# lorenzrichter/path-space-PDE-solver

Measured on AMD Instinct MI355X. Metric: trajectory-timesteps/sec (K*N/s), d=100 HJB log-variance training iteration, higher is better.
Workload: dtype f32 (f16x3 split products: every matrix product as three f16 MFMAs, fp32 accumulate; state / sums fp32)

## Files before the change

path-space-pde-solver_amd/csrc/hjb_basis_kernels.h:

```cpp
#pragma once
#include <hip/hip_runtime.h>

namespace psp {

constexpr int kBasisThreads = 256, kBasisRows = 4;
inline int basis_lds_bytes(int d) { return (kBasisRows * (d + 1) + d * d) * 4; }

template <bool TRANSPOSE>
__global__ __launch_bounds__(kBasisThreads) void hjb_basis_w1_kernel(const float* src, float* dst, const float* __restrict__ B,
                                                                     int d, int H, long long n) {
    extern __shared__ __attribute__((aligned(16))) float lds[];
    const int tid = threadIdx.x, nthr = blockDim.x;
    const int h0 = blockIdx.x * kBasisRows;
    const int rows = (H - h0) < kBasisRows ? (H - h0) : kBasisRows;
    const int nw = rows * (d + 1);
    const float* wsrc = src + (long long)h0 * (d + 1);
    float* wdst = dst + (long long)h0 * (d + 1);
    float* w = lds;
    float* m = lds + kBasisRows * (d + 1);
    for (int idx = tid; idx < nw; idx += nthr) w[idx] = wsrc[idx];
    for (int idx = tid; idx < d * d; idx += nthr) {
        const int i = idx / d, j = idx - i * d;
        m[TRANSPOSE ? j * d + i : idx] = B[idx];
    }
    if (dst != src) {
        const long long base = (long long)H * (d + 1);
        for (long long idx = base + (long long)blockIdx.x * nthr + tid; idx < n; idx += (long long)gridDim.x * nthr) dst[idx] = src[idx];
    }
    __syncthreads();
    for (int idx = tid; idx < nw; idx += nthr) {
        const int h = idx / (d + 1), c = idx - h * (d + 1);
        float v = w[idx];
        if (c > 0) {
            const float* row = w + h * (d + 1) + 1;
            const int j = c - 1;
            v = 0.f;
            for (int i = 0; i < d; ++i) v = fmaf(row[i], m[i * d + j], v);
        }
        wdst[idx] = v;
    }
}

template <bool TRANSPOSE>
inline hipError_t launch_basis_w1(const float* src, float* dst, const float* B, int d, int H, long long n, hipStream_t s) {
    const int grid = (H + kBasisRows - 1) / kBasisRows;
    hipLaunchKernelGGL((hjb_basis_w1_kernel<TRANSPOSE>), dim3(grid), dim3(kBasisThreads), basis_lds_bytes(d), s, src, dst, B, d, H, n);
    return hipGetLastError();
}

}
```

path-space-pde-solver_amd/csrc/hjb_kernels.h:

```cpp
#pragma once
#include <cstdlib>
#include <type_traits>
#include <hip/hip_runtime.h>
#include <stdint.h>

namespace psp {

typedef float f32x4 __attribute__((ext_vector_type(4)));

struct HjbArgs {
    const float* params;
    const float* x0;
    const float* y0;
    const float* xi;
    float* path;
    float* D;
    float* XN;
    double* fwd_partial;
    const float* drift;
    const float* sigma;
    const float* runcost;
    const float* term;
    const double* sums;
    float* grad_partial;
// ... 493 lines not shown
        split4c(last, b4h, b4l);
#pragma unroll
        for (int mb = 0; mb < MB; ++mb) {
            const f16x4* p = reinterpret_cast<const f16x4*>(wlds + mb * SG::per_mb + NS * 512) + lane;
            const f16x4 a_hi = p[0], a_lo = p[64];
            acc[mb] = __builtin_amdgcn_mfma_f32_16x16x16f16(a_hi, b4h, acc[mb], 0, 0, 0);
            corr[mb] = __builtin_amdgcn_mfma_f32_16x16x16f16(a_hi, b4l, corr[mb], 0, 0, 0);
            corr[mb] = __builtin_amdgcn_mfma_f32_16x16x16f16(a_lo, b4h, corr[mb], 0, 0, 0);
        }
    }
#pragma unroll
    for (int mb = 0; mb < MB; ++mb) acc[mb] = acc[mb] + kSplitInv * corr[mb];
}

__device__ __forceinline__ float qsum(float v) {
    v += __shfl_xor(v, 16);
    v += __shfl_xor(v, 32);
    return v;
}
__device__ __forceinline__ float jsumf(float v) {
    v += __shfl_xor(v, 1);
    v += __shfl_xor(v, 2);
    v += __shfl_xor(v, 4);
    v += __shfl_xor(v, 8);
    return v;
}
__device__ __forceinline__ double jsum(double v) {
    v += __shfl_xor(v, 1);
    v += __shfl_xor(v, 2);
    v += __shfl_xor(v, 4);
    v += __shfl_xor(v, 8);
    return v;
}

__device__ __forceinline__ float tanh_f32(float x) {
    const float e = __builtin_amdgcn_exp2f(fabsf(x) * 2.8853900817779268f);
    const float big = fmaf(-2.0f, __builtin_amdgcn_rcpf(e + 1.0f), 1.0f);
    return copysignf(big, x);
}
__device__ __forceinline__ f32x4 tanh4(f32x4 v) {
    f32x4 o;
    o[0] = tanh_f32(v[0]); o[1] = tanh_f32(v[1]); o[2] = tanh_f32(v[2]); o[3] = tanh_f32(v[3]);
    return o;
}

__device__ __forceinline__ f32x4 relu4n(f32x4 v) {
    f32x4 o;
    o[0] = v[0] < 0.f ? 0.f : v[0]; o[1] = v[1] < 0.f ? 0.f : v[1]; o[2] = v[2] < 0.f ? 0.f : v[2]; o[3] = v[3] < 0.f ? 0.f : v[3];
    return o;
}

template <int D, int H>
struct Geo {
    static constexpr int DB = cdiv(D, 16), HB = cdiv(H, 16);
    static constexpr int KSD = cdiv(D, 4), KSH = cdiv(H, 4);
    static constexpr int oW1 = 0, ob1 = H * (D + 1), oW2 = ob1 + H, ob2 = oW2 + H * H, oW3 = ob2 + H,
                         ob3 = oW3 + D * H, P = ob3 + D;
    static constexpr int fW1 = 0, fW2 = fW1 + HB * KSD * 64, fW3 = fW2 + HB * KSH * 64,
                         fVec = fW3 + DB * KSH * 64;
    static constexpr int vb1 = fVec, vw1t = vb1 + HB * 16, vb2 = vw1t + HB * 16, vb3 = vb2 + HB * 16,
                         vdr = vb3 + DB * 16, vrun = vdr + DB * 16, vterm = vrun + DB * 16,
                         fRed = vterm + DB * 16;
    static constexpr int fA = fRed + 64;
    static constexpr int fB_dense_off = DB * KSD * 64;
    static constexpr int xW1 = 0, xW2 = xW1 + SplitGeo<KSD, DB>::floats(HB), xW3 = xW2 + SplitGeo<KSH, HB>::floats(HB),
                         xVec = xW3 + SplitGeo<KSH, HB>::floats(DB), xA = xVec + (fA - fVec);
    static constexpr int xB_dense_off = SplitGeo<KSD, DB>::floats(DB);
    static int fwd_x3_lds_floats(int drift_kind, int sigma_kind) {
        return xA + (drift_kind == DRIFT_DENSE ? xB_dense_off : 0) + (sigma_kind == SIGMA_DENSE ? xB_dense_off : 0);
    }
    static int fwd_lds_floats(int drift_kind, int sigma_kind) {
        return fA + (drift_kind == DRIFT_DENSE ? fB_dense_off : 0) + (sigma_kind == SIGMA_DENSE ? fB_dense_off : 0);
    }
    static constexpr int pX = 0, pH1 = 4 * DB * 64, pH2 = pH1 + 4 * HB * 64, pXi = pH2 + 4 * HB * 64, PB = pXi + 4 * DB * 64;
    static constexpr int WH = (HB >= 4) ? 4 : (HB >= 2 ? 2 : 1);
    static constexpr int WD = 4 / WH;
    static constexpr int NIB = cdiv(HB, WH);
    static constexpr int NOBD = cdiv(DB, WD);
    static constexpr int NOBH = cdiv(HB, WD);
    static constexpr int EXB = KSD * 64 + 4 * HB * 64;
    static int bwd2_lds_floats() { return HB * KSD * 64 + 2 * 4 * EXB; }
};

template <int D, int H, int MODE = 0, int FAST_ = 0>
__global__ __launch_bounds__(512) void hjb_fwd_kernel(const HjbArgs a) {
    PSP_COND_EXIT(a);
    constexpr bool FAST = FAST_ != 0, SPEC = FAST_ >= 2;
    const int k_drift = SPEC ? (int)DRIFT_DENSE : a.drift_kind;
    const int k_sigma = FAST_ == 3 ? (int)SIGMA_IDENT : SPEC ? (int)SIGMA_DENSE : a.sigma_kind;
    const int k_run = SPEC ? (int)RUN_ZERO : a.runcost_kind, k_loss = SPEC ? (int)LOSS_LOGVAR : a.loss_kind;
    const int k_store = a.store_path;
    const bool k_adaptive = SPEC ? true : (a.adaptive != 0);
    const uint32_t iter_now = a.iter_dev ? *a.iter_dev : a.iter;
    using G = Geo<D, H>;
    constexpr int DB = G::DB, HB = G::HB, KSD = G::KSD, KSH = G::KSH;
    constexpr bool BF16 = MODE == 1, X3 = MODE == 2;
    constexpr int oW1 = X3 ? G::xW1 : G::fW1, oW2 = X3 ? G::xW2 : G::fW2, oW3 = X3 ? G::xW3 : G::fW3;
    constexpr int VEC = X3 ? G::xVec : G::fVec;
    constexpr int VSH = VEC - G::fVec;
    extern __shared__ __attribute__((aligned(16))) float lds[];
    const int tid = threadIdx.x, nthr = blockDim.x;
    const int lane = tid & 63, wave = tid >> 6, nwave = nthr >> 6;
    const int j = lane & 15, q = lane >> 4;

    const float* __restrict__ P = a.params;
    auto stage_net = [&](float* dst, int MB, int KS, int INB, auto src) {
        if constexpr (BF16) stage_aop_bf16(dst, MB, (INB + 1) / 2, tid, nthr, src);
        else stage_aop(dst, MB, KS, tid, nthr, src);
    };
    auto w1src = [&](int row, int col) { return (row < H && col < D) ? P[G::oW1 + row * (D + 1) + 1 + col] : 0.f; };
    auto w2src = [&](int row, int col) { return (row < H && col < H) ? P[G::oW2 + row * H + col] : 0.f; };
    auto w3src = [&](int row, int col) { return (row < D && col < H) ? P[G::oW3 + row * H + col] : 0.f; };
    if constexpr (X3) {
        stage_aop_x3<KSD, DB>(lds + oW1, HB, tid, nthr, w1src);
        stage_aop_x3<KSH, HB>(lds + oW2, HB, tid, nthr, w2src);
        stage_aop_x3<KSH, HB>(lds + oW3, DB, tid, nthr, w3src);
    } else {
        stage_net(lds + oW1, HB, KSD, DB, w1src);
        stage_net(lds + oW2, HB, KSH, HB, w2src);
        stage_net(lds + oW3, DB, KSH, HB, w3src);
    }
    float* ldsA = lds + G::fA + VSH;
    float* ldsB = ldsA + (k_drift == DRIFT_DENSE ? (X3 ? G::xB_dense_off : G::fB_dense_off) : 0);
    if (k_drift == DRIFT_DENSE) {
        const float dt = a.dt;
        const float* __restrict__ A = a.drift;
        auto asrc = [&](int row, int col) { return (row < D && col < D) ? dt * A[row * D + col] : 0.f; };
        if constexpr (X3) stage_aop_x3<KSD, DB>(ldsA, DB, tid, nthr, asrc);
        else stage_aop(ldsA, DB, KSD, tid, nthr, asrc);
    }
    if (k_sigma == SIGMA_DENSE) {
        const float* __restrict__ B = a.sigma;
        auto bsrc = [&](int row, int col) { return (row < D && col < D) ? B[row * D + col] : 0.f; };
        if constexpr (X3) stage_aop_x3<KSD, DB>(ldsB, DB, tid, nthr, bsrc);
        else stage_aop(ldsB, DB, KSD, tid, nthr, bsrc);
    }
    stage_vec(lds + VSH + G::vb1, HB, tid, nthr, [&](int f) { return f < H ? P[G::ob1 + f] : 0.f; });
    stage_vec(lds + VSH + G::vw1t, HB, tid, nthr, [&](int f) { return f < H ? P[G::oW1 + f * (D + 1)] : 0.f; });
    stage_vec(lds + VSH + G::vb2, HB, tid, nthr, [&](int f) { return f < H ? P[G::ob2 + f] : 0.f; });
    stage_vec(lds + VSH + G::vb3, DB, tid, nthr, [&](int f) { return f < D ? P[G::ob3 + f] : 0.f; });
    stage_vec(lds + VSH + G::vdr, DB, tid, nthr, [&](int f) {
        return (f < D && (k_drift == DRIFT_DIAG || k_drift == DRIFT_DWELL)) ? a.drift[f] : 0.f; });
    stage_vec(lds + VSH + G::vrun, DB, tid, nthr, [&](int f) {
        return (f < D && k_run == RUN_DIAGQ) ? a.runcost[f] : 0.f; });
    stage_vec(lds + VSH + G::vterm, DB, tid, nthr, [&](int f) { return f < D ? a.term[f] : 0.f; });
    __syncthreads();

    const int t16 = blockIdx.x * nwave + wave;
    const bool wave_valid = t16 < a.ntile16;
    const int k = t16 * 16 + j;
    const bool kvalid = wave_valid && k < a.K_local;
    const uint32_t kglob = (uint32_t)(a.k_offset + k);
    const float dt = a.dt, sqdt = a.sqdt;

    const float store_cxi = SPEC ? 1.f : ((k_store == 3) ? 0.f : 1.f);
    const float store_cz = SPEC ? 0.f : ((k_store == 3) ? 1.f : (k_store == 2 ? -a.sqdt : (k_adaptive ? 0.f : a.sqdt)));
    const bool do_store = FAST ? true : (k_store != 0);
    double sD = 0.0, sD2 = 0.0;
    if (wave_valid) {
        const f32x4* vecs0 = reinterpret_cast<const f32x4*>(lds + VEC) + q;
        const f32x4* vterm = vecs0 + (G::vterm - G::fVec) / 4;

        f32x4 X[DB];
#pragma unroll
        for (int b = 0; b < DB; ++b) {
#pragma unroll
            for (int r = 0; r < 4; ++r) {
                const int f = 16 * b + 4 * r + q;
                const float v = a.x0[(size_t)(kvalid ? k : 0) * a.x0_stride + (f < D ? f : D - 1)];
                X[b][r] = (f < D && kvalid) ? v : 0.f;
            }
        }
        float Y = a.y0 ? a.y0[0] : 0.f;
        float Fsum = 0.f, ULsum = 0.f;
#ifdef PSP_STAMPS
        unsigned long long stamps[8] = {0, 0, 0, 0, 0, 0, 0, 0};
#endif

        for (int n = 0; n < a.N; ++n) {
            PSP_STAMP(fs0);
            float tn = (float)n * dt;
            if constexpr (!FAST) { if (a.tfeat) tn = a.tfeat[n]; }
            const f32x4* vecs = opaque(vecs0);
            const f32x4* vb1 = vecs + (G::vb1 - G::fVec) / 4;
            const f32x4* vw1t = vecs + (G::vw1t - G::fVec) / 4;
            const f32x4* vb2 = vecs + (G::vb2 - G::fVec) / 4;
            const f32x4* vb3 = vecs + (G::vb3 - G::fVec) / 4;
            const f32x4* vdr = vecs + (G::vdr - G::fVec) / 4;
            const f32x4* vrun = vecs + (G::vrun - G::fVec) / 4;
            float* pblk = a.path + ((size_t)n * a.ntile16 + t16) * (size_t)G::PB + lane;
            auto x_store = [&](int u, int NU) __attribute__((always_inline)) {
                if (do_store) {
#pragma unroll
                    for (int ks = 0; ks < 4 * DB; ++ks)
                        if (ks >= u * (4 * DB) / NU && ks < (u + 1) * (4 * DB) / NU)
                            PSP_PATH_STORE(pblk + (G::pX / 64 + ks) * 64, X[ks >> 2][ks & 3]);
                }
            };
            if (!X3 && do_store) {
#pragma unroll
                for (int ks = 0; ks < 4 * DB; ++ks) PSP_PATH_STORE(pblk + (G::pX / 64 + ks) * 64, X[ks >> 2][ks & 3]);
            }
            f32x4 h1[HB];
#pragma unroll
            for (int m = 0; m < HB; ++m) h1[m] = vb1[m * 4] + tn * vw1t[m * 4];
            f32x4 Tn[DB];
            const bool early_drift = X3 && k_drift == DRIFT_DENSE;
            if constexpr (X3) {
                if (k_drift == DRIFT_DENSE) {
                    f16x8 xh[DB / 2 > 0 ? DB / 2 : 1], xl[DB / 2 > 0 ? DB / 2 : 1];
                    constexpr int NU1 = (DB / 2) * HB, NU2 = (DB / 2) * DB;
                    split_panel8<DB>(X, xh, xl);
                    gemm_Txs<HB, KSD, DB, 2>(h1, lds + oW1, xh, xl, X[DB - 1], lane, [&](int u) __attribute__((always_inline)) { x_store(u, NU1 + NU2); });
#pragma unroll
                    for (int b = 0; b < DB; ++b) Tn[b] = X[b];
                    gemm_Txs<DB, KSD, DB, 2>(Tn, ldsA, xh, xl, X[DB - 1], lane, [&](int u) __attribute__((always_inline)) { x_store(NU1 + u, NU1 + NU2); });
                    if constexpr (NU1 + NU2 == 0) x_store(0, 1);
                } else {
                    constexpr int NU1 = (DB / 2) * HB;
                    gemm_Tx<HB, KSD, DB, 2>(h1, lds + oW1, X, lane, [&](int u) __attribute__((always_inline)) { x_store(u, NU1); });
                    if constexpr (NU1 == 0) x_store(0, 1);
                }
            }
            else if constexpr (BF16) gemm_Tb<HB, DB>(h1, lds + oW1, X, lane);
            else gemm_T<HB, KSD, DB>(h1, lds + oW1, X, lane);
            PSP_STAMP(fs1);
#pragma unroll
            for (int m = 0; m < HB; ++m) h1[m] = tanh4(h1[m]);
            PSP_STAMP(fs2);
            f32x4 h2[HB];
#pragma unroll
            for (int m = 0; m < HB; ++m) h2[m] = vb2[m * 4];
            constexpr int NUH2 = (HB / 2) * HB, NUH3 = (HB / 2) * DB;
            constexpr bool PREGEN = X3 && FAST && (NUH2 + NUH3 > 0);
            [[maybe_unused]] f32x4 xig[PREGEN ? DB : 1];
            [[maybe_unused]] uint32_t pc0 = 0, pc1 = 0, pc2 = 0, pc3 = 0;
            constexpr int NSPC = kPhiloxRounds + 1;
            auto philox_slice = [&](int sidx) __attribute__((always_inline)) {
                const int b = sidx / NSPC, sub = sidx % NSPC;
                if (sub == 0) { pc0 = kglob; pc1 = (uint32_t)n; pc2 = (uint32_t)(4 * b + q); pc3 = iter_now; }
                if (sub < kPhiloxRounds) {
                    philox_round(pc0, pc1, pc2, pc3, a.seed_lo + (uint32_t)sub * 0x9E3779B9u, a.seed_hi + (uint32_t)sub * 0xBB67AE85u);
                    asm volatile("" : "+v"(pc0), "+v"(pc1), "+v"(pc2), "+v"(pc3));
                } else {
                    const uint32_t rr[4] = {pc0, pc1, pc2, pc3};
                    f32x4 xi = normal4(rr);
                    if (16 * b + 16 > D) {
#pragma unroll
                        for (int r = 0; r < 4; ++r) if (16 * b + 4 * r + q >= D) xi[r] = 0.f;
                    }
                    asm volatile("" : "+v"(xi));
                    xig[b < DB ? b : 0] = xi;
                }
            };
            auto philox_portion = [&](int u) __attribute__((always_inline)) {
                if constexpr (PREGEN) {
#pragma unroll
                    for (int sidx = 0; sidx < NSPC * DB; ++sidx)
                        if (sidx >= u * (NSPC * DB) / (NUH2 + NUH3) && sidx < (u + 1) * (NSPC * DB) / (NUH2 + NUH3)) philox_slice(sidx);
                }
            };
            auto h_store = [&](const f32x4 (&h)[HB], int slot, int u, int NU) __attribute__((always_inline)) {
                if (do_store) {
#pragma unroll
                    for (int ks = 0; ks < 4 * HB; ++ks)
                        if (ks >= u * (4 * HB) / NU && ks < (u + 1) * (4 * HB) / NU)
                            PSP_PATH_STORE(pblk + (slot / 64 + ks) * 64, h[ks >> 2][ks & 3]);
                }
            };
            if constexpr (X3) {
                gemm_Tx<HB, KSH, HB, 2>(h2, lds + oW2, h1, lane, [&](int u) __attribute__((always_inline)) { h_store(h1, G::pH1, u, NUH2); philox_portion(u); });
                if constexpr (NUH2 == 0) h_store(h1, G::pH1, 0, 1);
            }
            else if constexpr (BF16) gemm_Tb<HB, HB>(h2, lds + oW2, h1, lane);
            else gemm_T<HB, KSH, HB>(h2, lds + oW2, h1, lane);
#pragma unroll
            for (int m = 0; m < HB; ++m) h2[m] = tanh4(h2[m]);
            if (!X3 && do_store) {
#pragma unroll
                for (int ks = 0; ks < 4 * HB; ++ks) {
                    PSP_PATH_STORE(pblk + (G::pH1 / 64 + ks) * 64, h1[ks >> 2][ks & 3]);
                    PSP_PATH_STORE(pblk + (G::pH2 / 64 + ks) * 64, h2[ks >> 2][ks & 3]);
                }
            }
            f32x4 Z[DB];
#pragma unroll
            for (int m = 0; m < DB; ++m) Z[m] = vb3[m * 4];
            if constexpr (X3) {
                gemm_Tx<DB, KSH, HB, 2>(Z, lds + oW3, h2, lane, [&](int u) __attribute__((always_inline)) { h_store(h2, G::pH2, u, NUH3); philox_portion(NUH2 + u); });
                if constexpr (NUH3 == 0) h_store(h2, G::pH2, 0, 1);
            }
            else if constexpr (BF16) gemm_Tb<DB, HB>(Z, lds + oW3, h2, lane);
            else gemm_T<DB, KSH, HB>(Z, lds + oW3, h2, lane);
            PSP_STAMP(fs3);

            float S = 0.f, Pz = 0.f, UL = 0.f;
#pragma unroll
            for (int b = 0; b < DB; ++b) {
                f32x4 xi;
                if constexpr (PREGEN) {
                    xi = xig[b];
                } else if (FAST || a.noise_mode == NOISE_PHILOX) {
                    xi = philox_block(kglob, (uint32_t)n, (uint32_t)(4 * b + q), iter_now, a.seed_lo, a.seed_hi);
                } else {
                    const float* xrow = a.xi + ((size_t)(n + 1) * a.K_local + (kvalid ? k : 0)) * D;
#pragma unroll
                    for (int r = 0; r < 4; ++r) {
                        const int f = 16 * b + 4 * r + q;
                        const float v = xrow[f < D ? f : D - 1];
                        xi[r] = (f < D && kvalid) ? v : 0.f;
                    }
                }
                if (16 * b + 16 > D) {
#pragma unroll
                    for (int r = 0; r < 4; ++r) if (16 * b + 4 * r + q >= D) xi[r] = 0.f;
                }
                if (do_store && k_store != 4) {
                    const f32x4 wv = store_cxi * xi + store_cz * Z[b];
#pragma unroll
                    for (int r = 0; r < 4; ++r) PSP_PATH_STORE(pblk + (G::pXi / 64 + 4 * b + r) * 64, wv[r]);
                }
#pragma unroll
                for (int r = 0; r < 4; ++r) {
                    S = fmaf(Z[b][r], Z[b][r], S);
                    Pz = fmaf(Z[b][r], xi[r], Pz);
                }
                if (!FAST && a.uref) {
                    const float* ur = a.uref + (size_t)n * D;
#pragma unroll
                    for (int r = 0; r < 4; ++r) {
                        const int f = 16 * b + 4 * r + q;
                        const float e = (f < D) ? Z[b][r] + ur[f < D ? f : D - 1] : 0.f;
                        UL = fmaf(e, e, UL);
                    }
                }
                Z[b] = k_adaptive ? (sqdt * xi - dt * Z[b]) : (sqdt * xi);
            }
            ULsum = fmaf(UL, dt, ULsum);
            S = qsum(S);
            Pz = qsum(Pz);
            PSP_STAMP(fs4);

            if (!early_drift) {
#pragma unroll
                for (int b = 0; b < DB; ++b) Tn[b] = X[b];
            }
            if (k_drift == DRIFT_DENSE) {
                if constexpr (!X3) gemm_T<DB, KSD, DB>(Tn, ldsA, X, lane);
            } else if (k_drift == DRIFT_DIAG) {
#pragma unroll
                for (int b = 0; b < DB; ++b) Tn[b] += dt * (vdr[b * 4] * X[b]);
            } else if (k_drift == DRIFT_DWELL) {
#pragma unroll
                for (int b = 0; b < DB; ++b) Tn[b] -= dt * (4.0f * vdr[b * 4] * (X[b] * (X[b] * X[b] - 1.0f)));
            }
            if (k_sigma == SIGMA_DENSE) {
                if constexpr (X3) gemm_Tx<DB, KSD, DB>(Tn, ldsB, Z, lane);
                else gemm_T<DB, KSD, DB>(Tn, ldsB, Z, lane);
            } else if (k_sigma == SIGMA_SCALE) {
#pragma unroll
                for (int b = 0; b < DB; ++b) Tn[b] += a.sigma_scale * Z[b];
            } else {
#pragma unroll
                for (int b = 0; b < DB; ++b) Tn[b] += Z[b];
            }
#pragma unroll
            for (int b = 0; b < DB; ++b) X[b] = Tn[b];
            PSP_STAMP(fs5);

            float fX = 0.f;
            if (k_run == RUN_DIAGQ) {
#pragma unroll
                for (int b = 0; b < DB; ++b) {
                    const f32x4 pv = vrun[b * 4];
#pragma unroll
                    for (int r = 0; r < 4; ++r) fX = fmaf(pv[r] * X[b][r], X[b][r], fX);
                }
                fX = qsum(fX);
            }
            if (k_loss == LOSS_RELENT) {
                Y = Y - (0.5f * S + fX) * dt;
            } else {
                const float drift_y = k_adaptive ? (fX - 0.5f * S) : (fX + 0.5f * S);
                Y = Y + drift_y * dt + Pz * sqdt;
            }
            Fsum = fmaf(fX, dt, Fsum);
            PSP_STAMP(fs6);
            PSP_ACC(0, fs1, fs0);
            PSP_ACC(1, fs2, fs1);
            PSP_ACC(2, fs3, fs2);
            PSP_ACC(3, fs4, fs3);
            PSP_ACC(4, fs5, fs4);
            PSP_ACC(5, fs6, fs5);
            PSP_ACC(6, fs6, fs0);
        }
#ifdef PSP_STAMPS
        if (a.dbg && lane == 0) {
            stamps[7] = (unsigned long long)a.N;
            for (int i = 0; i < 8; ++i) a.dbg[((size_t)blockIdx.x * 8 + wave) * 8 + i] = stamps[i];
// ... 493 lines not shown
```

path-space-pde-solver_amd/csrc/hjbx_kernels.h:

```cpp
#pragma once
#include "hjb_kernels.h"

namespace psp {

template <int D, int H>
struct GeoX {
    using G = Geo<D, H>;
    static constexpr int DB = G::DB, HB = G::HB, KSD = G::KSD, KSH = G::KSH;
    static constexpr int T3 = 0, T2 = T3 + SplitGeo<KSD, DB>::floats(HB), EX = T2 + SplitGeo<KSH, HB>::floats(HB);
    static constexpr int hG = 0, hGl = hG + D * 32, hZ2 = hGl + D * 32, hZ2l = hZ2 + HB * 512, hZ1 = hZ2l + HB * 512,
                         hZ1l = hZ1 + HB * 512, PAIRH = hZ1l + HB * 512;
    static constexpr int RS = 16 * DB + 3 * 16 * HB;
    static constexpr int NX = cdiv(DB, 4);
    static constexpr int NT = DB + 2 * HB;
    static_assert(4 * RS <= 4 * (PAIRH / 2), "bias sums reuse the exchange area");
    static constexpr int GS = EX + 4 * (PAIRH / 2);
    static int lds_floats() { return GS + 12; }
};

template <int NB>
__device__ __forceinline__ void split_panel(const f32x4 (&v)[NB], f16x4 (&hi)[NB], f16x4 (&lo)[NB]) {
#pragma unroll
    for (int b = 0; b < NB; ++b) {
        if ((NB & 1) && b == NB - 1) split4c(v[b], hi[b], lo[b]);
        else split4(v[b], hi[b], lo[b]);
    }
}

template <int MB, int KS, int INB>
__device__ __forceinline__ void gemm_Txp(f32x4 (&acc)[MB], const float* wlds, const f16x4 (&hi)[INB], const f16x4 (&lo)[INB],
                                         float last, int lane) {
    using SG = SplitGeo<KS, INB>;
    constexpr int NS = SG::NS;
    lane = opaque_i(lane);
    f32x4 corr[MB];
#pragma unroll
    for (int mb = 0; mb < MB; ++mb) corr[mb] = f32x4{0.f, 0.f, 0.f, 0.f};
    if constexpr (NS > 0) {
        const f16x8* tbl = reinterpret_cast<const f16x8*>(wlds) + lane;
        constexpr int NU = NS * MB, CU = 1, NCH = cdiv(NU, CU);
        f16x8 ah[2][CU], al[2][CU];
#pragma unroll
        for (int kk = 0; kk < CU; ++kk)
            if (kk < NU) {
                ah[0][kk] = tbl[((kk % MB) * SG::per_mb + (kk / MB) * 512) / 4];
                al[0][kk] = tbl[((kk % MB) * SG::per_mb + (kk / MB) * 512) / 4 + 64];
            }
#pragma unroll
        for (int c = 0; c < NCH; ++c) {
            if (c + 1 < NCH) {
#pragma unroll
                for (int kk = 0; kk < CU; ++kk) {
                    const int u = (c + 1) * CU + kk;
                    if (u < NU) {
                        ah[(c + 1) & 1][kk] = tbl[((u % MB) * SG::per_mb + (u / MB) * 512) / 4];
                        al[(c + 1) & 1][kk] = tbl[((u % MB) * SG::per_mb + (u / MB) * 512) / 4 + 64];
                    }
                }
            }
#pragma unroll
            for (int kk = 0; kk < CU; ++kk) {
                const int u = c * CU + kk;
                if (u < NU) {
                    const int S = u / MB, mb = u % MB;
                    const f16x8 bh = __builtin_shufflevector(hi[2 * S], hi[2 * S + 1], 0, 1, 2, 3, 4, 5, 6, 7);
                    const f16x8 bl = __builtin_shufflevector(lo[2 * S], lo[2 * S + 1], 0, 1, 2, 3, 4, 5, 6, 7);
                    acc[mb] = __builtin_amdgcn_mfma_f32_16x16x32_f16(ah[c & 1][kk], bh, acc[mb], 0, 0, 0);
                    corr[mb] = __builtin_amdgcn_mfma_f32_16x16x32_f16(ah[c & 1][kk], bl, corr[mb], 0, 0, 0);
                    corr[mb] = __builtin_amdgcn_mfma_f32_16x16x32_f16(al[c & 1][kk], bh, corr[mb], 0, 0, 0);
                }
            }
            __builtin_amdgcn_sched_barrier(kFenceMask);
        }
    }
    if constexpr (SG::ODD_F32) {
#pragma unroll
        for (int mb = 0; mb < MB; ++mb) acc[mb] = mfma16(wlds[mb * SG::per_mb + NS * 512 + lane], last, acc[mb]);
    }
    if constexpr (SG::ODD_H16) {
#pragma unroll
        for (int mb = 0; mb < MB; ++mb) {
            const f16x4* p = reinterpret_cast<const f16x4*>(wlds + mb * SG::per_mb + NS * 512) + lane;
            const f16x4 a_hi = p[0], a_lo = p[64];
            acc[mb] = __builtin_amdgcn_mfma_f32_16x16x16f16(a_hi, hi[INB - 1], acc[mb], 0, 0, 0);
            corr[mb] = __builtin_amdgcn_mfma_f32_16x16x16f16(a_hi, lo[INB - 1], corr[mb], 0, 0, 0);
            corr[mb] = __builtin_amdgcn_mfma_f32_16x16x16f16(a_lo, hi[INB - 1], corr[mb], 0, 0, 0);
        }
    }
#pragma unroll
    for (int mb = 0; mb < MB; ++mb) acc[mb] = acc[mb] + kSplitInv * corr[mb];
}

template <int D, int H, bool REGEN = false>
__global__ __launch_bounds__(512) void hjb_bwd3_kernel(const HjbArgs a) {
    PSP_COND_EXIT(a);
    GradCheck<true> gchk;
    using G = Geo<D, H>;
    using X = GeoX<D, H>;
    constexpr int DB = G::DB, HB = G::HB, KSD = G::KSD, KSH = G::KSH, NX = X::NX, RS = X::RS, PAIRH = X::PAIRH, NT = X::NT;
    extern __shared__ __attribute__((aligned(16))) float lds[];
    const int tid = threadIdx.x, nthr = blockDim.x;
    const int lane = tid & 63, wave = __builtin_amdgcn_readfirstlane(tid >> 6);
    const int j = lane & 15, q = lane >> 4;
    const bool producer = wave < 4;
    const int sub = wave & 3;
    const float* __restrict__ P = a.params;

    const double invK = 1.0 / (double)a.K_global;
    const float meanD = (a.loss_kind == LOSS_LOGVAR) ? (float)(a.sums[0] * invK) : 0.f;
    const float coef = (float)(2.0 * invK);
    {
        float wm = 0.f;
        for (int k = tid; k < a.K_local; k += nthr) {
            const float dk = a.D[k];
            wm = fmaxf(wm, fabsf(a.loss_kind == LOSS_WEIGHTS ? dk : coef * (dk - meanD)));
        }
#pragma unroll
        for (int o = 1; o < 64; o <<= 1) wm = fmaxf(wm, __shfl_xor(wm, o));
        if (lane == 0) lds[X::GS + 4 + wave] = wm;
    }
    stage_aop_x3<KSD, DB>(lds + X::T3, HB, tid, nthr, [&](int row, int col) {
        return (row < H && col < D) ? P[G::oW3 + col * H + row] : 0.f; });
    stage_aop_x3<KSH, HB>(lds + X::T2, HB, tid, nthr, [&](int row, int col) {
        return (row < H && col < H) ? P[G::oW2 + col * H + row] : 0.f; });
    __syncthreads();
    _Float16* exh = reinterpret_cast<_Float16*>(lds + X::EX);
    const bool xi_image = a.adaptive != 0 && (a.store_path == 1 || a.store_path == 4);
    auto g_scale = [&](float& gs, float& ginv) __attribute__((always_inline)) {
        const float* slot = lds + X::GS;
        float imax = fmaxf(fmaxf(slot[0], slot[1]), fmaxf(slot[2], slot[3]));
        if (xi_image || !(imax >= 1.1754944e-38f)) imax = xi_image ? 8.0f : 1.0f;
        const float wmax = fmaxf(fmaxf(fmaxf(slot[4], slot[5]), fmaxf(slot[6], slot[7])),
                                 fmaxf(fmaxf(slot[8], slot[9]), fmaxf(slot[10], slot[11])));
        const float amax = wmax * a.sqdt * imax;
        const unsigned e = (__float_as_uint(amax) >> 23) & 0xFFu;
        const bool ok = e >= 1u && e <= 253u;
        gs = ok ? __uint_as_float((254u - e) << 23) : 1.0f;
        ginv = ok ? __uint_as_float(e << 23) : 1.0f;
    };
    const f32x4 zero4 = {0.f, 0.f, 0.f, 0.f};
    const float sqdt = a.sqdt, dt = a.dt;
    constexpr bool regen = REGEN;
    const uint32_t iter_now = a.iter_dev ? *a.iter_dev : a.iter;
    const long long nblk = (long long)a.N * a.ntile16;
    const long long nround = (nblk + 3) / 4;
    const int R = (int)((nround - blockIdx.x + gridDim.x - 1) / gridDim.x);

    if (producer) {
        f32x4 sG[DB], sZ2[HB], sZ1[HB], sT1[HB];
#pragma unroll
        for (int b = 0; b < DB; ++b) sG[b] = zero4;
#pragma unroll
        for (int m = 0; m < HB; ++m) { sZ2[m] = zero4; sZ1[m] = zero4; sT1[m] = zero4; }
        auto own_block = [&](int it2) __attribute__((always_inline)) {
            const long long b0 = ((long long)blockIdx.x + (long long)it2 * gridDim.x) * 4 + sub;
            return b0 < nblk ? b0 : -1LL;
        };
        auto path_of = [&](int it2) __attribute__((always_inline)) {
            const long long b0 = own_block(it2);
            return a.path + (size_t)(b0 >= 0 ? b0 : nblk - 1) * (size_t)G::PB + lane;
        };
        f32x4 xin[DB], h2n[HB], h1n[HB];
        float dkn;
        {
            const long long b0 = own_block(0);
            const long long blk = b0 >= 0 ? b0 : nblk - 1;
            const float* pb = path_of(0);
            const int k0 = (int)(blk % a.ntile16) * 16 + j;
            dkn = a.D[k0 < a.K_local ? k0 : 0];
            if constexpr (regen) {
#pragma unroll
                for (int b = 0; b < DB; ++b) xin[b] = zero4;
            } else {
#pragma unroll
                for (int b = 0; b < DB; ++b)
#pragma unroll
                    for (int r = 0; r < 4; ++r) xin[b][r] = pb[G::pXi + (4 * b + r) * 64];
            }
            if constexpr (regen) {
#pragma unroll
                for (int m = 0; m < HB; ++m)
#pragma unroll
                    for (int r = 0; r < 4; ++r) h2n[m][r] = pb[G::pH2 + (4 * m + r) * 64];
#pragma unroll
                for (int m = 0; m < HB; ++m)
#pragma unroll
                    for (int r = 0; r < 4; ++r) h1n[m][r] = pb[G::pH1 + (4 * m + r) * 64];
            }
        }
        float gs, ginv;
        {
            const long long b0 = own_block(0);
            const int k0 = (int)((b0 >= 0 ? b0 : nblk - 1) % a.ntile16) * 16 + j;
            const bool kv = b0 >= 0 && k0 < a.K_local;
            float am = 0.f;
#pragma unroll
            for (int b = 0; b < DB; ++b)
#pragma unroll
                for (int r = 0; r < 4; ++r) am = fmaxf(am, kv ? fabsf(xin[b][r]) : 0.f);
#pragma unroll
            for (int o = 1; o < 64; o <<= 1) am = fmaxf(am, __shfl_xor(am, o));
            if (lane == 0) lds[X::GS + sub] = am;
            __syncthreads();
            g_scale(gs, ginv);
        }
#ifdef PSP_STAMPS
        unsigned long long stamps[8] = {0, 0, 0, 0, 0, 0, 0, 0};
#endif
        for (int it = 0; it <= R; ++it) {
            PSP_STAMP(tp0);
            if (it < R) {
                const long long blk0 = own_block(it);
                const bool bvalid = blk0 >= 0;
                const long long blk = bvalid ? blk0 : nblk - 1;
                const int t16 = (int)(blk % a.ntile16);
                const int k = t16 * 16 + j;
                const bool kvalid = bvalid && k < a.K_local;
                const float tn = (float)(blk / a.ntile16) * dt;
                _Float16* ex0 = exh + ((it & 1) * 2 + (sub >> 1)) * PAIRH + (sub & 1) * 4 + (j & 3);
                _Float16* exr[4] = {ex0 + (((j >> 2) ^ 0) * 8), ex0 + (((j >> 2) ^ 1) * 8), ex0 + (((j >> 2) ^ 2) * 8), ex0 + (((j >> 2) ^ 3) * 8)};
                const float* pn = path_of(it + 1);
                const float* pc = path_of(it);
                const float dkc = dkn;
                if constexpr (!regen) {
#pragma unroll
                    for (int m = 0; m < HB; ++m)
#pragma unroll
                        for (int r = 0; r < 4; ++r) h2n[m][r] = pc[G::pH2 + (4 * m + r) * 64];
                }
                const float wk = kvalid ? (a.loss_kind == LOSS_WEIGHTS ? dkc : coef * (dkc - meanD)) : 0.f;
                f32x4 Gt[DB];
                if constexpr (regen) {
                    const uint32_t kg = (uint32_t)(a.k_offset + k), nstep = (uint32_t)(blk / a.ntile16);
                    const int qo = opaque_i(q);
#pragma unroll
                    for (int b = 0; b < DB; ++b) {
                        f32x4 xi = philox_block(kg, nstep, (uint32_t)(4 * b + qo), iter_now, a.seed_lo, a.seed_hi);
                        if (16 * b + 16 > D) {
#pragma unroll
                            for (int r = 0; r < 4; ++r) if (16 * b + 4 * r + q >= D) xi[r] = 0.f;
                        }
                        {
#pragma clang fp contract(off)
                            Gt[b] = (wk * sqdt * gs) * xi;
                            sG[b] += Gt[b];
                        }
                        __builtin_amdgcn_sched_barrier(0);
                    }
                } else {
                    {
#pragma clang fp contract(off)
#pragma unroll
                        for (int b = 0; b < DB; ++b) {
                            Gt[b] = (wk * sqdt * gs) * xin[b];
                            sG[b] += Gt[b];
                        }
                    }
                }
                PSP_STAMP(tp1);
                PSP_ACC(0, tp1, tp0);
                f16x4 Gh[DB], Gl[DB];
                split_panel<DB>(Gt, Gh, Gl);
#pragma unroll
                for (int b = 0; b < DB; ++b)
#pragma unroll
                    for (int r = 0; r < 4; ++r) {
                        const int f = 16 * b + 4 * r + q;
                        if (16 * b + 16 <= D || f < D) {
                            exr[r][X::hG + f * 32] = Gh[b][r];
                            exr[r][X::hGl + f * 32] = Gl[b][r];
                        }
                    }
                PSP_STAMP(tp2);
                PSP_ACC(1, tp2, tp1);
                f32x4 dz2[HB];
#pragma unroll
                for (int m = 0; m < HB; ++m) dz2[m] = zero4;
                gemm_Txp<HB, KSD, DB>(dz2, lds + X::T3, Gh, Gl, Gt[DB - 1][0], lane);
                {
#pragma clang fp contract(off)
#pragma unroll
                    for (int m = 0; m < HB; ++m) { dz2[m] = dz2[m] * (1.0f - h2n[m] * h2n[m]); sZ2[m] += dz2[m]; }
                }
                if constexpr (regen) {
                    __builtin_amdgcn_sched_barrier(0);
#pragma unroll
                    for (int m = 0; m < HB; ++m)
#pragma unroll
                        for (int r = 0; r < 4; ++r) h2n[m][r] = pn[G::pH2 + (4 * m + r) * 64];
                } else {
#pragma unroll
                    for (int m = 0; m < HB; ++m)
#pragma unroll
                        for (int r = 0; r < 4; ++r) h1n[m][r] = pc[G::pH1 + (4 * m + r) * 64];
                    const long long n0 = own_block(it + 1);
                    const long long nb1 = n0 >= 0 ? n0 : nblk - 1;
                    const int k1 = (int)(nb1 % a.ntile16) * 16 + j;
                    dkn = a.D[k1 < a.K_local ? k1 : 0];
#pragma unroll
                    for (int b = 0; b < DB; ++b)
#pragma unroll
                        for (int r = 0; r < 4; ++r) xin[b][r] = pn[G::pXi + (4 * b + r) * 64];
                }
                PSP_STAMP(tp3);
                PSP_ACC(2, tp3, tp2);
                f16x4 Zh[HB], Zl[HB];
                split_panel<HB>(dz2, Zh, Zl);
#pragma unroll
                for (int m = 0; m < HB; ++m)
#pragma unroll
                    for (int r = 0; r < 4; ++r) {
                        exr[r][X::hZ2 + (16 * m + 4 * r + q) * 32] = Zh[m][r];
                        exr[r][X::hZ2l + (16 * m + 4 * r + q) * 32] = Zl[m][r];
                    }
                f32x4 dz1[HB];
#pragma unroll
                for (int m = 0; m < HB; ++m) dz1[m] = zero4;
                gemm_Txp<HB, KSH, HB>(dz1, lds + X::T2, Zh, Zl, dz2[HB - 1][0], lane);
                {
#pragma clang fp contract(off)
#pragma unroll
                    for (int m = 0; m < HB; ++m) {
                        dz1[m] = dz1[m] * (1.0f - h1n[m] * h1n[m]);
                        sZ1[m] += dz1[m];
                        sT1[m] += tn * dz1[m];
                    }
                }
                if constexpr (regen) {
                    __builtin_amdgcn_sched_barrier(0);
                    const long long n0 = own_block(it + 1);
                    const long long nb1 = n0 >= 0 ? n0 : nblk - 1;
                    const int k1 = (int)(nb1 % a.ntile16) * 16 + j;
                    dkn = a.D[k1 < a.K_local ? k1 : 0];
#pragma unroll
                    for (int m = 0; m < HB; ++m)
#pragma unroll
                        for (int r = 0; r < 4; ++r) h1n[m][r] = pn[G::pH1 + (4 * m + r) * 64];
                }
                split_panel<HB>(dz1, Zh, Zl);
#pragma unroll
                for (int m = 0; m < HB; ++m)
#pragma unroll
                    for (int r = 0; r < 4; ++r) {
                        exr[r][X::hZ1 + (16 * m + 4 * r + q) * 32] = Zh[m][r];
                        exr[r][X::hZ1l + (16 * m + 4 * r + q) * 32] = Zl[m][r];
                    }
            }
            PSP_STAMP(tp4);
            PSP_ACC(3, tp4, tp0);
            __syncthreads();
            PSP_STAMP(tp5);
            PSP_ACC(4, tp5, tp4);
            PSP_ACC(6, tp5, tp0);
        }
#ifdef PSP_STAMPS
        if (a.dbg && lane == 0) {
            stamps[7] = (unsigned long long)R;
            for (int i = 0; i < 8; ++i) a.dbg[((size_t)blockIdx.x * 8 + wave) * 8 + i] = stamps[i];
        }
#endif
        float* red = lds + X::EX + sub * RS;
#pragma unroll
        for (int b = 0; b < DB; ++b)
#pragma unroll
            for (int r = 0; r < 4; ++r) {
                const float v = ginv * jsumf(sG[b][r]);
                if (j == 0) red[16 * b + 4 * r + q] = v;
            }
#pragma unroll
        for (int m = 0; m < HB; ++m)
#pragma unroll
            for (int r = 0; r < 4; ++r) {
                const float v2 = ginv * jsumf(sZ2[m][r]), v1 = ginv * jsumf(sZ1[m][r]), vt = ginv * jsumf(sT1[m][r]);
                if (j == 0) {
                    red[16 * DB + 16 * m + 4 * r + q] = v2;
                    red[16 * DB + 16 * HB + 16 * m + 4 * r + q] = v1;
                    red[16 * DB + 32 * HB + 16 * m + 4 * r + q] = vt;
                }
            }
        __syncthreads();
        return;
    }
    const int ibw = sub < HB ? sub : HB - 1;
    int obx[NX];
#pragma unroll
    for (int s = 0; s < NX; ++s) obx[s] = (sub + 4 * s) < DB ? (sub + 4 * s) : DB - 1;
    f32x4 a3[DB], a2[HB], a1[HB][NX], c1[HB][NX];
#pragma unroll
    for (int b = 0; b < DB; ++b) a3[b] = zero4;
#pragma unroll
    for (int m = 0; m < HB; ++m) {
        a2[m] = zero4;
#pragma unroll
        for (int s = 0; s < NX; ++s) { a1[m][s] = zero4; c1[m][s] = zero4; }
    }
    const int nblk_i = (int)nblk;
    auto blk_at = [&](long long c0) __attribute__((always_inline)) {
        const int c = (c0 < (long long)nblk_i) ? (int)c0 : nblk_i - 1;
        return __builtin_amdgcn_readfirstlane(c);
    };
    typedef const __attribute__((address_space(1))) float* gptr_t;
    auto sbase = [&](int blk, int ofs) __attribute__((always_inline)) {
        return (gptr_t)sgpr_block_addr(a.path, (unsigned long long)blk, (unsigned)G::PB, (unsigned)ofs);
    };
    const unsigned lofsU = (unsigned)image_lane_offset_F(lane);
    auto get_F = [&](gptr_t base) __attribute__((always_inline)) {
        return *reinterpret_cast<const __attribute__((address_space(1))) f32x4*>(base + lofsU);
    };
    f32x4 Lh2[2], Lh1[2], Lx[NX][2];
    auto issue = [&](int c0, int c1) __attribute__((always_inline)) {
        Lh2[0] = get_F(sbase(c0, G::pH2 + ibw * 256)); Lh2[1] = get_F(sbase(c1, G::pH2 + ibw * 256));
        Lh1[0] = get_F(sbase(c0, G::pH1 + ibw * 256)); Lh1[1] = get_F(sbase(c1, G::pH1 + ibw * 256));
#pragma unroll
        for (int s = 0; s < NX; ++s) {
            Lx[s][0] = get_F(sbase(c0, G::pX + obx[s] * 256));
            Lx[s][1] = get_F(sbase(c1, G::pX + obx[s] * 256));
        }
    };
    auto pack = [&](const f32x4& u0, const f32x4& u1, f16x8& hi, f16x8& lo) __attribute__((always_inline)) {
        split8(u0, u1, hi, lo);
    };
    const int aofs = opaque_i((lane & 15) * 32 + (((lane >> 4) ^ ((lane >> 2) & 3)) * 8));
    auto a_load = [&](const _Float16* e, int t, f16x8& Ah, f16x8& Al) __attribute__((always_inline)) {
        const int hi = t < DB ? X::hG + t * 512 : (t < DB + HB ? X::hZ2 + (t - DB) * 512 : X::hZ1 + (t - DB - HB) * 512);
        const int lo = t < DB ? X::hGl + t * 512 : (t < DB + HB ? X::hZ2l + (t - DB) * 512 : X::hZ1l + (t - DB - HB) * 512);
        Ah = *reinterpret_cast<const f16x8*>(e + hi + aofs);
        Al = *reinterpret_cast<const f16x8*>(e + lo + aofs);
    };
    const f16x8 k2048 = {(_Float16)2048.f, (_Float16)2048.f, (_Float16)2048.f, (_Float16)2048.f,
                         (_Float16)2048.f, (_Float16)2048.f, (_Float16)2048.f, (_Float16)2048.f};
    auto pair_phase = [&](const _Float16* e, int n0, int n1) __attribute__((always_inline)) {
        f16x8 Ah[3], Al[3];
        a_load(e, 0, Ah[0], Al[0]);
        a_load(e, 1, Ah[1], Al[1]);
        f16x8 h2h, h2l, h1h, h1l, xh[NX], xl[NX];
        pack(Lh2[0], Lh2[1], h2h, h2l);
        pack(Lh1[0], Lh1[1], h1h, h1l);
#pragma unroll
        for (int s = 0; s < NX; ++s) pack(Lx[s][0], Lx[s][1], xh[s], xl[s]);
        const f16x8 h2s = h2h * k2048, h1s = h1h * k2048;
        __builtin_amdgcn_sched_barrier(0);
        issue(n0, n1);
        __builtin_amdgcn_sched_barrier(0);
#pragma unroll
        for (int t = 0; t < NT; ++t) {
            if (t + 2 < NT) a_load(e, t + 2, Ah[(t + 2) % 3], Al[(t + 2) % 3]);
            const f16x8 ah = Ah[t % 3], al = Al[t % 3];
            if (t < DB) {
                a3[t] = __builtin_amdgcn_mfma_f32_16x16x32_f16(ah, h2s, a3[t], 0, 0, 0);
                a3[t] = __builtin_amdgcn_mfma_f32_16x16x32_f16(ah, h2l, a3[t], 0, 0, 0);
                a3[t] = __builtin_amdgcn_mfma_f32_16x16x32_f16(al, h2h, a3[t], 0, 0, 0);
            } else if (t < DB + HB) {
                const int m = t - DB;
                a2[m] = __builtin_amdgcn_mfma_f32_16x16x32_f16(ah, h1s, a2[m], 0, 0, 0);
                a2[m] = __builtin_amdgcn_mfma_f32_16x16x32_f16(ah, h1l, a2[m], 0, 0, 0);
                a2[m] = __builtin_amdgcn_mfma_f32_16x16x32_f16(al, h1h, a2[m], 0, 0, 0);
            } else {
                const int m = t - DB - HB;
#pragma unroll
                for (int s = 0; s < NX; ++s) {
                    a1[m][s] = __builtin_amdgcn_mfma_f32_16x16x32_f16(ah, xh[s], a1[m][s], 0, 0, 0);
                    c1[m][s] = __builtin_amdgcn_mfma_f32_16x16x32_f16(ah, xl[s], c1[m][s], 0, 0, 0);
                    c1[m][s] = __builtin_amdgcn_mfma_f32_16x16x32_f16(al, xh[s], c1[m][s], 0, 0, 0);
                }
            }
            __builtin_amdgcn_sched_barrier(kFenceMask);
        }
    };

    {
        const long long rb = (long long)blockIdx.x * 4;
        issue(blk_at(rb), blk_at(rb + 1));
    }
    __syncthreads();
    __syncthreads();
#ifdef PSP_STAMPS
    unsigned long long stamps[8] = {0, 0, 0, 0, 0, 0, 0, 0};
#endif
    for (int it = 1; it <= R; ++it) {
        PSP_STAMP(tc0);
        const long long rb = ((long long)blockIdx.x + (long long)(it - 1) * gridDim.x) * 4;
        const _Float16* exr = exh + ((it - 1) & 1) * 2 * PAIRH;
        const long long rn = rb + 4LL * gridDim.x;
        pair_phase(exr, blk_at(rb + 2), blk_at(rb + 3));
        PSP_STAMP(tc1);
        pair_phase(exr + PAIRH, blk_at(rn), blk_at(rn + 1));
        PSP_STAMP(tc2);
        PSP_ACC(0, tc2, tc0);
        PSP_ACC(1, tc1, tc0);
        __syncthreads();
        PSP_STAMP(tc3);
        PSP_ACC(4, tc3, tc2);
        PSP_ACC(6, tc3, tc0);
    }
#ifdef PSP_STAMPS
    if (a.dbg && lane == 0) {
        stamps[7] = (unsigned long long)R;
        for (int i = 0; i < 8; ++i) a.dbg[((size_t)blockIdx.x * 8 + wave) * 8 + i] = stamps[i];
    }
#endif
    float gs, ginv;
    g_scale(gs, ginv);
    const float inv1 = ginv, inv2 = ginv * kSplitInv;

    float* gp = a.grad_partial + (size_t)blockIdx.x * G::P;
    const int col = lane & 15, qq = lane >> 4;
    if (sub < HB) {
#pragma unroll
        for (int b = 0; b < DB; ++b) {
            const f32x4 v = inv2 * a3[b];
#pragma unroll
            for (int rr = 0; rr < 4; ++rr) {
                const int o3 = 16 * b + 4 * qq + rr, i3 = 16 * sub + col;
                if (o3 < D && i3 < H) { const float gv_ = v[rr]; gp[G::oW3 + o3 * H + i3] = gv_; gchk.see(gv_); }
            }
        }
#pragma unroll
        for (int m = 0; m < HB; ++m) {
            const f32x4 v = inv2 * a2[m];
#pragma unroll
            for (int rr = 0; rr < 4; ++rr) {
                const int o2 = 16 * m + 4 * qq + rr, i2 = 16 * sub + col;
                if (o2 < H && i2 < H) { const float gv_ = v[rr]; gp[G::oW2 + o2 * H + i2] = gv_; gchk.see(gv_); }
            }
        }
    }
#pragma unroll
    for (int m = 0; m < HB; ++m)
#pragma unroll
        for (int s = 0; s < NX; ++s) {
            const f32x4 v = inv1 * (a1[m][s] + kSplitInv * c1[m][s]);
            const int ob = sub + 4 * s;
#pragma unroll
            for (int rr = 0; rr < 4; ++rr) {
                const int o1 = 16 * m + 4 * qq + rr, i1 = 16 * ob + col;
                if (ob < DB && o1 < H && i1 < D) { const float gv_ = v[rr]; gp[G::oW1 + o1 * (D + 1) + 1 + i1] = gv_; gchk.see(gv_); }
            }
        }
    __syncthreads();
    {
        const float* red = lds + X::EX;
        const int ct = tid - 256;
        for (int f = ct; f < D; f += 256)
            { const float gv_ = (red[f] + red[RS + f]) + (red[2 * RS + f] + red[3 * RS + f]); gp[G::ob3 + f] = gv_; gchk.see(gv_); }
        for (int f = ct; f < H; f += 256) {
            const float* r2 = red + 16 * DB + f;
            { const float gv_ = (r2[0] + r2[RS]) + (r2[2 * RS] + r2[3 * RS]); gp[G::ob2 + f] = gv_; gchk.see(gv_); }
            const float* r1 = r2 + 16 * HB;
            { const float gv_ = (r1[0] + r1[RS]) + (r1[2 * RS] + r1[3 * RS]); gp[G::ob1 + f] = gv_; gchk.see(gv_); }
            const float* rt = r1 + 16 * HB;
            { const float gv_ = (rt[0] + rt[RS]) + (rt[2 * RS] + rt[3 * RS]); gp[G::oW1 + f * (D + 1)] = gv_; gchk.see(gv_); }
        }
    }
    gchk.raise(a.cond);
}

template <int D, int H>
struct HjbxLaunch {
    using X = GeoX<D, H>;
    static int lds_bytes() { return X::lds_floats() * 4; }
    static hipError_t bwd(const HjbArgs& a, int grid, hipStream_t s) {
        const int bytes = lds_bytes();
        if (a.store_path == 4) {
            hipError_t e = hipFuncSetAttribute(reinterpret_cast<const void*>(&hjb_bwd3_kernel<D, H, true>),
                                               hipFuncAttributeMaxDynamicSharedMemorySize, bytes);
            if (e != hipSuccess) return e;
            hipLaunchKernelGGL((hjb_bwd3_kernel<D, H, true>), dim3(grid), dim3(512), bytes, s, a);
            return hipGetLastError();
        }
        hipError_t e = hipFuncSetAttribute(reinterpret_cast<const void*>(&hjb_bwd3_kernel<D, H, false>),
                                           hipFuncAttributeMaxDynamicSharedMemorySize, bytes);
        if (e != hipSuccess) return e;
        hipLaunchKernelGGL((hjb_bwd3_kernel<D, H, false>), dim3(grid), dim3(512), bytes, s, a);
        return hipGetLastError();
    }
};

}
```

Before: 1.773 billion.

## Reuse padding slots of stored path for noise tail and bias/time gradient

The path buffer's unused padded x rows now carry the final noise block's values, or a constant 1 and time feature row. The backward kernel reads those instead of regenerating Philox noise for the last block, and obtains the b1 and time-weight gradients directly from the W1 MFMA accumulation instead of separate per-step sums and reductions. The basis transform kernel is also reworked to one row per block with a padded transposed matrix stride to avoid LDS bank conflicts. This adds layout coupling between the forward store and the backward read, and relies on the padded slots being otherwise unused.

Result: no change. 1.778 billion, median of 6 (+0.2%).

```diff
diff --git a/path-space-pde-solver_amd/csrc/hjb_basis_kernels.h b/path-space-pde-solver_amd/csrc/hjb_basis_kernels.h
--- a/path-space-pde-solver_amd/csrc/hjb_basis_kernels.h
+++ b/path-space-pde-solver_amd/csrc/hjb_basis_kernels.h
@@ -3,48 +3,49 @@
 
 namespace psp {
 
-constexpr int kBasisThreads = 256, kBasisRows = 4;
-inline int basis_lds_bytes(int d) { return (kBasisRows * (d + 1) + d * d) * 4; }
+constexpr int kBasisThreads = 256;
+inline int basis_row_stride(int d) { return d | 1; }
+inline int basis_lds_bytes(int d) { return ((d + 1) + d * basis_row_stride(d)) * 4; }
 
 template <bool TRANSPOSE>
 __global__ __launch_bounds__(kBasisThreads) void hjb_basis_w1_kernel(const float* src, float* dst, const float* __restrict__ B,
                                                                      int d, int H, long long n) {
     extern __shared__ __attribute__((aligned(16))) float lds[];
     const int tid = threadIdx.x, nthr = blockDim.x;
-    const int h0 = blockIdx.x * kBasisRows;
-    const int rows = (H - h0) < kBasisRows ? (H - h0) : kBasisRows;
-    const int nw = rows * (d + 1);
-    const float* wsrc = src + (long long)h0 * (d + 1);
-    float* wdst = dst + (long long)h0 * (d + 1);
+    const int h = blockIdx.x;
+    const int ld = TRANSPOSE ? (d | 1) : d;
+    const float* wsrc = src + (long long)h * (d + 1);
+    float* wdst = dst + (long long)h * (d + 1);
     float* w = lds;
-    float* m = lds + kBasisRows * (d + 1);
-    for (int idx = tid; idx < nw; idx += nthr) w[idx] = wsrc[idx];
-    for (int idx = tid; idx < d * d; idx += nthr) {
-        const int i = idx / d, j = idx - i * d;
-        m[TRANSPOSE ? j * d + i : idx] = B[idx];
+    float* m = lds + (d + 1);
+    for (int idx = tid; idx <= d; idx += nthr) w[idx] = wsrc[idx];
+    if (TRANSPOSE) {
+        for (int r = tid >> 6; r < d; r += nthr >> 6)
+            for (int c = tid & 63; c < d; c += 64) m[r * ld + c] = B[r * d + c];
+    } else {
+        for (int idx = tid; idx < d * d; idx += nthr) m[idx] = B[idx];
     }
     if (dst != src) {
         const long long base = (long long)H * (d + 1);
         for (long long idx = base + (long long)blockIdx.x * nthr + tid; idx < n; idx += (long long)gridDim.x * nthr) dst[idx] = src[idx];
     }
     __syncthreads();
-    for (int idx = tid; idx < nw; idx += nthr) {
-        const int h = idx / (d + 1), c = idx - h * (d + 1);
-        float v = w[idx];
+    for (int c = tid; c <= d; c += nthr) {
+        float v = w[c];
         if (c > 0) {
-            const float* row = w + h * (d + 1) + 1;
             const int j = c - 1;
+            const float* col = TRANSPOSE ? m + j * ld : m + j;
+            const int step = TRANSPOSE ? 1 : d;
             v = 0.f;
-            for (int i = 0; i < d; ++i) v = fmaf(row[i], m[i * d + j], v);
+            for (int i = 0; i < d; ++i) v = fmaf(w[1 + i], col[i * step], v);
         }
-        wdst[idx] = v;
+        wdst[c] = v;
     }
 }
 
 template <bool TRANSPOSE>
 inline hipError_t launch_basis_w1(const float* src, float* dst, const float* B, int d, int H, long long n, hipStream_t s) {
-    const int grid = (H + kBasisRows - 1) / kBasisRows;
-    hipLaunchKernelGGL((hjb_basis_w1_kernel<TRANSPOSE>), dim3(grid), dim3(kBasisThreads), basis_lds_bytes(d), s, src, dst, B, d, H, n);
+    hipLaunchKernelGGL((hjb_basis_w1_kernel<TRANSPOSE>), dim3(H), dim3(kBasisThreads), basis_lds_bytes(d), s, src, dst, B, d, H, n);
     return hipGetLastError();
 }
 
diff --git a/path-space-pde-solver_amd/csrc/hjb_kernels.h b/path-space-pde-solver_amd/csrc/hjb_kernels.h
--- a/path-space-pde-solver_amd/csrc/hjb_kernels.h
+++ b/path-space-pde-solver_amd/csrc/hjb_kernels.h
@@ -599,6 +599,15 @@
     static int bwd2_lds_floats() { return HB * KSD * 64 + 2 * 4 * EXB; }
 };
 
+template <int D>
+struct PadSlots {
+    static constexpr int DB = cdiv(D, 16), NR = cdiv(D - 16 * (DB - 1), 4);
+    static constexpr bool TAIL = 2 * NR <= 4;
+    static constexpr int RA = TAIL ? 2 * NR : NR;
+    static constexpr bool AUX = RA < 4;
+    static constexpr int ksT = 4 * (DB - 1) + NR, ksA = 4 * (DB - 1) + RA;
+};
+
 template <int D, int H, int MODE = 0, int FAST_ = 0>
 __global__ __launch_bounds__(512) void hjb_fwd_kernel(const HjbArgs a) {
     PSP_COND_EXIT(a);
@@ -615,6 +624,8 @@
     constexpr int oW1 = X3 ? G::xW1 : G::fW1, oW2 = X3 ? G::xW2 : G::fW2, oW3 = X3 ? G::xW3 : G::fW3;
     constexpr int VEC = X3 ? G::xVec : G::fVec;
     constexpr int VSH = VEC - G::fVec;
+    using PS = PadSlots<D>;
+    constexpr bool TAIL = X3 && PS::TAIL, AUX = X3 && PS::AUX;
     extern __shared__ __attribute__((aligned(16))) float lds[];
     const int tid = threadIdx.x, nthr = blockDim.x;
     const int lane = tid & 63, wave = tid >> 6, nwave = nthr >> 6;
@@ -710,8 +721,20 @@
                 if (do_store) {
 #pragma unroll
                     for (int ks = 0; ks < 4 * DB; ++ks)
-                        if (ks >= u * (4 * DB) / NU && ks < (u + 1) * (4 * DB) / NU)
-                            PSP_PATH_STORE(pblk + (G::pX / 64 + ks) * 64, X[ks >> 2][ks & 3]);
+                        if (ks >= u * (4 * DB) / NU && ks < (u + 1) * (4 * DB) / NU) {
+                            if (TAIL && ks >= PS::ksT && ks < PS::ksT + PS::NR) continue;
+                            if (AUX && ks == PS::ksA) {
+                                const int qa = (int)__builtin_amdgcn_mbcnt_hi(~0u, __builtin_amdgcn_mbcnt_lo(~0u, (unsigned)opaque_i(0))) >> 4;
+                                PSP_PATH_STORE(pblk + (G::pX / 64 + ks) * 64, qa == 0 ? 1.0f : (qa == 1 ? (float)n * dt : 0.f));
+                            } else
+                                PSP_PATH_STORE(pblk + (G::pX / 64 + ks) * 64, X[ks >> 2][ks & 3]);
+                        }
+                }
+            };
+            auto tail_store = [&](const f32x4& xi) __attribute__((always_inline)) {
+                if (do_store) {
+#pragma unroll
+                    for (int r = 0; r < PS::NR; ++r) PSP_PATH_STORE(pblk + (G::pX / 64 + PS::ksT + r) * 64, xi[r]);
                 }
             };
             if (!X3 && do_store) {
@@ -768,6 +791,7 @@
                     }
                     asm volatile("" : "+v"(xi));
                     xig[b < DB ? b : 0] = xi;
+                    if constexpr (TAIL) { if (b == DB - 1) tail_store(xi); }
                 }
             };
             auto philox_portion = [&](int u) __attribute__((always_inline)) {
@@ -832,6 +856,7 @@
 #pragma unroll
                     for (int r = 0; r < 4; ++r) if (16 * b + 4 * r + q >= D) xi[r] = 0.f;
                 }
+                if constexpr (TAIL && !PREGEN) { if (b == DB - 1) tail_store(xi); }
                 if (do_store && k_store != 4) {
                     const f32x4 wv = store_cxi * xi + store_cz * Z[b];
 #pragma unroll
diff --git a/path-space-pde-solver_amd/csrc/hjbx_kernels.h b/path-space-pde-solver_amd/csrc/hjbx_kernels.h
--- a/path-space-pde-solver_amd/csrc/hjbx_kernels.h
+++ b/path-space-pde-solver_amd/csrc/hjbx_kernels.h
@@ -97,7 +97,9 @@
     GradCheck<true> gchk;
     using G = Geo<D, H>;
     using X = GeoX<D, H>;
+    using PS = PadSlots<D>;
     constexpr int DB = G::DB, HB = G::HB, KSD = G::KSD, KSH = G::KSH, NX = X::NX, RS = X::RS, PAIRH = X::PAIRH, NT = X::NT;
+    constexpr bool TAIL = REGEN && PS::TAIL, AUX = PS::AUX;
     extern __shared__ __attribute__((aligned(16))) float lds[];
     const int tid = threadIdx.x, nthr = blockDim.x;
     const int lane = tid & 63, wave = __builtin_amdgcn_readfirstlane(tid >> 6);
@@ -161,6 +163,7 @@
             return a.path + (size_t)(b0 >= 0 ? b0 : nblk - 1) * (size_t)G::PB + lane;
         };
         f32x4 xin[DB], h2n[HB], h1n[HB];
+        [[maybe_unused]] float xtn[PS::NR];
         float dkn;
         {
             const long long b0 = own_block(0);
@@ -168,6 +171,10 @@
             const float* pb = path_of(0);
             const int k0 = (int)(blk % a.ntile16) * 16 + j;
             dkn = a.D[k0 < a.K_local ? k0 : 0];
+            if constexpr (TAIL) {
+#pragma unroll
+                for (int r = 0; r < PS::NR; ++r) xtn[r] = pb[G::pX + (PS::ksT + r) * 64];
+            }
             if constexpr (regen) {
 #pragma unroll
                 for (int b = 0; b < DB; ++b) xin[b] = zero4;
@@ -235,10 +242,17 @@
                     const int qo = opaque_i(q);
 #pragma unroll
                     for (int b = 0; b < DB; ++b) {
-                        f32x4 xi = philox_block(kg, nstep, (uint32_t)(4 * b + qo), iter_now, a.seed_lo, a.seed_hi);
-                        if (16 * b + 16 > D) {
-#pragma unroll
-                            for (int r = 0; r < 4; ++r) if (16 * b + 4 * r + q >= D) xi[r] = 0.f;
+                        f32x4 xi;
+                        if (TAIL && b == DB - 1) {
+                            xi = zero4;
+#pragma unroll
+                            for (int r = 0; r < PS::NR; ++r) xi[r] = xtn[r];
+                        } else {
+                            xi = philox_block(kg, nstep, (uint32_t)(4 * b + qo), iter_now, a.seed_lo, a.seed_hi);
+                            if (16 * b + 16 > D) {
+#pragma unroll
+                                for (int r = 0; r < 4; ++r) if (16 * b + 4 * r + q >= D) xi[r] = 0.f;
+                            }
                         }
                         {
 #pragma clang fp contract(off)
@@ -284,6 +298,10 @@
                 }
                 if constexpr (regen) {
                     __builtin_amdgcn_sched_barrier(0);
+                    if constexpr (TAIL) {
+#pragma unroll
+                        for (int r = 0; r < PS::NR; ++r) xtn[r] = pn[G::pX + (PS::ksT + r) * 64];
+                    }
 #pragma unroll
                     for (int m = 0; m < HB; ++m)
 #pragma unroll
@@ -322,8 +340,10 @@
 #pragma unroll
                     for (int m = 0; m < HB; ++m) {
                         dz1[m] = dz1[m] * (1.0f - h1n[m] * h1n[m]);
-                        sZ1[m] += dz1[m];
-                        sT1[m] += tn * dz1[m];
+                        if constexpr (!AUX) {
+                            sZ1[m] += dz1[m];
+                            sT1[m] += tn * dz1[m];
+                        }
                     }
                 }
                 if constexpr (regen) {
@@ -371,11 +391,14 @@
         for (int m = 0; m < HB; ++m)
 #pragma unroll
             for (int r = 0; r < 4; ++r) {
-                const float v2 = ginv * jsumf(sZ2[m][r]), v1 = ginv * jsumf(sZ1[m][r]), vt = ginv * jsumf(sT1[m][r]);
-                if (j == 0) {
-                    red[16 * DB + 16 * m + 4 * r + q] = v2;
-                    red[16 * DB + 16 * HB + 16 * m + 4 * r + q] = v1;
-                    red[16 * DB + 32 * HB + 16 * m + 4 * r + q] = vt;
+                const float v2 = ginv * jsumf(sZ2[m][r]);
+                if (j == 0) red[16 * DB + 16 * m + 4 * r + q] = v2;
+                if constexpr (!AUX) {
+                    const float v1 = ginv * jsumf(sZ1[m][r]), vt = ginv * jsumf(sT1[m][r]);
+                    if (j == 0) {
+                        red[16 * DB + 16 * HB + 16 * m + 4 * r + q] = v1;
+                        red[16 * DB + 32 * HB + 16 * m + 4 * r + q] = vt;
+                    }
                 }
             }
         __syncthreads();
@@ -504,7 +527,8 @@
     const float inv1 = ginv, inv2 = ginv * kSplitInv;
 
     float* gp = a.grad_partial + (size_t)blockIdx.x * G::P;
-    const int col = lane & 15, qq = lane >> 4;
+    const int lane_e = (int)__builtin_amdgcn_mbcnt_hi(~0u, __builtin_amdgcn_mbcnt_lo(~0u, 0u));
+    const int col = lane_e & 15, qq = lane_e >> 4;
     if (sub < HB) {
 #pragma unroll
         for (int b = 0; b < DB; ++b) {
@@ -535,21 +559,30 @@
             for (int rr = 0; rr < 4; ++rr) {
                 const int o1 = 16 * m + 4 * qq + rr, i1 = 16 * ob + col;
                 if (ob < DB && o1 < H && i1 < D) { const float gv_ = v[rr]; gp[G::oW1 + o1 * (D + 1) + 1 + i1] = gv_; gchk.see(gv_); }
+                if constexpr (AUX) {
+                    if (ob == DB - 1 && o1 < H && (col == 4 * PS::RA || col == 4 * PS::RA + 1)) {
+                        const float gv_ = v[rr];
+                        gp[col == 4 * PS::RA ? G::ob1 + o1 : G::oW1 + o1 * (D + 1)] = gv_;
+                        gchk.see(gv_);
+                    }
+                }
             }
         }
     __syncthreads();
     {
         const float* red = lds + X::EX;
-        const int ct = tid - 256;
+        const int ct = sub * 64 + lane_e;
         for (int f = ct; f < D; f += 256)
             { const float gv_ = (red[f] + red[RS + f]) + (red[2 * RS + f] + red[3 * RS + f]); gp[G::ob3 + f] = gv_; gchk.see(gv_); }
         for (int f = ct; f < H; f += 256) {
             const float* r2 = red + 16 * DB + f;
             { const float gv_ = (r2[0] + r2[RS]) + (r2[2 * RS] + r2[3 * RS]); gp[G::ob2 + f] = gv_; gchk.see(gv_); }
-            const float* r1 = r2 + 16 * HB;
-            { const float gv_ = (r1[0] + r1[RS]) + (r1[2 * RS] + r1[3 * RS]); gp[G::ob1 + f] = gv_; gchk.see(gv_); }
-            const float* rt = r1 + 16 * HB;
-            { const float gv_ = (rt[0] + rt[RS]) + (rt[2 * RS] + rt[3 * RS]); gp[G::oW1 + f * (D + 1)] = gv_; gchk.see(gv_); }
+            if constexpr (!AUX) {
+                const float* r1 = r2 + 16 * HB;
+                { const float gv_ = (r1[0] + r1[RS]) + (r1[2 * RS] + r1[3 * RS]); gp[G::ob1 + f] = gv_; gchk.see(gv_); }
+                const float* rt = r1 + 16 * HB;
+                { const float gv_ = (rt[0] + rt[RS]) + (rt[2 * RS] + rt[3 * RS]); gp[G::oW1 + f * (D + 1)] = gv_; gchk.see(gv_); }
+            }
         }
     }
     gchk.raise(a.cond);
```
